# daniel05155/Reinforcement-Learning-in-Music-Generation

Measured on AMD Instinct MI355X. Metric: CW-tokens/sec pretrain fwd+bwd @T=1024, higher is better.
Workload: dtype bf16; 1 GPU; agent_pretrain step (fwd+bwd+clip+Adam), repo dims 512/12/8/2048, synthetic CW tokens (B=512/GPU, T=1024, 7 fields -> 6); per_gpu_batch=512, global_batch=512, seq_len=1024, parallelism=dp1, params=38982227, gemm_table=True

## Files before the change

reinforcement-learning-in-music-generation_amd/csrc/gemm_ln.hip:

```cpp
#include "cwlt_common.h"
#include "cwlt_lds_dma.h"
#include <stdlib.h>

namespace cwlt {
namespace gl {

constexpr int TMR = 128, TNC = 512, BK = 32;
constexpr int NSTAGE = 3;
constexpr int STG = (TMR + TNC) * BK * 2;
constexpr int LDE = TNC + 8;
constexpr int LDS_BYTES = TMR * LDE * 2 > NSTAGE * STG ? TMR * LDE * 2 : NSTAGE * STG;

typedef __bf16 bf16x4 __attribute__((ext_vector_type(4)));

__global__ __launch_bounds__(1024) void gemm_ln_kernel(
    const bf16_t* __restrict__ A, const bf16_t* __restrict__ W, const float* __restrict__ bias,
    const bf16_t* __restrict__ X, const float* __restrict__ gamma, const float* __restrict__ beta,
    bf16_t* __restrict__ S, bf16_t* __restrict__ Y, float* __restrict__ mean, float* __restrict__ rstd, long M, int K,
    long lda, long ldw, float eps, uint32_t thresh, float keep_scale, uint64_t seed,
    const uint64_t* __restrict__ seed_base) {
    extern __shared__ __attribute__((aligned(16))) char lds[];

    const int tid = threadIdx.x, lane = tid & 63;
    const int w = __builtin_amdgcn_readfirstlane(tid >> 6);
    const int wm = w >> 3, wn = w & 7;
    const int l31 = lane & 31, hf = lane >> 5;
    const long m0 = (long)blockIdx.x * TMR;
    const long mrows = min((long)TMR, M - m0);

    const uint64_t abase = (uint64_t)(A + m0 * lda), wbase = (uint64_t)W;
    u32x4_t ars, wrs;
    ars[0] = __builtin_amdgcn_readfirstlane((uint32_t)abase);
    ars[1] = __builtin_amdgcn_readfirstlane((uint32_t)(abase >> 32));
    ars[2] = __builtin_amdgcn_readfirstlane((uint32_t)(((mrows - 1) * lda + K) * 2));
    ars[3] = 0x00020000u;
    wrs[0] = __builtin_amdgcn_readfirstlane((uint32_t)wbase);
    wrs[1] = __builtin_amdgcn_readfirstlane((uint32_t)(wbase >> 32));
    wrs[2] = __builtin_amdgcn_readfirstlane((uint32_t)(((long)(TNC - 1) * ldw + K) * 2));
    wrs[3] = 0x00020000u;
    const int dchunk = (lane & 3) ^ ((lane >> 4) & 3);
    const uint32_t a_voff = ((uint32_t)(16 * (w & 7) + (lane >> 2)) * (uint32_t)lda + dchunk * 8) * 2;
    const uint32_t w_voff = ((uint32_t)(32 * w + (lane >> 2)) * (uint32_t)ldw + dchunk * 8) * 2;
    const uint32_t w_16 = (uint32_t)(16 * ldw * 2);
    const uint32_t lds_a = (uint32_t)(uintptr_t)(lds_void*)lds + (w & 7) * 1024;
    const uint32_t lds_w = (uint32_t)(uintptr_t)(lds_void*)lds + TMR * 64 + w * 2048;
#define GL_DMA_W(stage, step)                                                                                     \
    {                                                                                                             \
        unsigned keep;                                                                                            \
        const uint32_t lw = lds_w + (uint32_t)(stage) * STG;                                                      \
        const uint32_t sk_ = (uint32_t)(step) * (BK * 2), sk2 = sk_ + w_16;                                       \
        asm volatile("s_mov_b32 %0, m0\n\ts_mov_b32 m0, %2\n\ts_nop 4\n\t"                                     \
                     "buffer_load_dwordx4 %1, %3, %4 offen lds\n\t"                                               \
                     "s_add_u32 m0, %2, 0x400\n\ts_nop 0\n\t"                                                    \
                     "buffer_load_dwordx4 %1, %3, %5 offen lds\n\t"                                               \
                     "s_mov_b32 m0, %0"                                                                           \
                     : "=&s"(keep)                                                                                \
                     : "v"(w_voff), "s"(lw), "s"(wrs), "s"(sk_), "s"(sk2)                                         \
                     : "memory", "scc");                                                                          \
    }
#define GL_DMA_A(stage, step) lds_dma_piece(a_voff, ars, lds_a + (uint32_t)(stage) * STG, (uint32_t)(step) * (BK * 2))
#define GL_DMA(stage, step)        \
    {                              \
        if (w < 8) GL_DMA_A(stage, step); \
        GL_DMA_W(stage, step);     \
    }
    const int swz = (l31 >> 2) & 3;
    const int of0 = l31 * 64 + ((hf ^ swz) << 4), of1 = l31 * 64 + (((2 + hf) ^ swz) << 4);
    const int oa = (64 * wm) * 64, ow = TMR * 64 + (64 * wn) * 64;
#define GL_FRAG(p) __builtin_bit_cast(bf16x8, *reinterpret_cast<const uint4*>(p))
#define GL_READ(F, stage, ofh)                                            \
    {                                                                     \
        const char* sb = lds + (stage) * STG;                             \
        F[0] = GL_FRAG(sb + ow + (ofh));                                  \
        F[1] = GL_FRAG(sb + ow + 2048 + (ofh));                           \
        F[2] = GL_FRAG(sb + oa + (ofh));                                  \
        F[3] = GL_FRAG(sb + oa + 2048 + (ofh));                           \
    }
#define GL_MFMA(F)                                                                          \
    {                                                                                       \
        acc[0][0] = __builtin_amdgcn_mfma_f32_32x32x16_bf16(F[0], F[2], acc[0][0], 0, 0, 0); \
        acc[0][1] = __builtin_amdgcn_mfma_f32_32x32x16_bf16(F[1], F[2], acc[0][1], 0, 0, 0); \
        acc[1][0] = __builtin_amdgcn_mfma_f32_32x32x16_bf16(F[0], F[3], acc[1][0], 0, 0, 0); \
        acc[1][1] = __builtin_amdgcn_mfma_f32_32x32x16_bf16(F[1], F[3], acc[1][1], 0, 0, 0); \
    }

    f32x16 acc[2][2];
#pragma unroll
    for (int i = 0; i < 2; ++i)
#pragma unroll
        for (int j = 0; j < 2; ++j)
#pragma unroll
            for (int r = 0; r < 16; ++r) acc[i][j][r] = 0.f;

    const int nstep = K / BK;
    bf16x8 F0[4], F1[4];
    GL_DMA(0, 0);
    GL_DMA(1, 1);
    if (nstep > 2) GL_DMA(2, 2);
    if (nstep > 2) {
        if (w < 8)
            asm volatile("s_waitcnt vmcnt(6)" ::: "memory");
        else
            asm volatile("s_waitcnt vmcnt(4)" ::: "memory");
    } else {
        if (w < 8)
            asm volatile("s_waitcnt vmcnt(3)" ::: "memory");
        else
            asm volatile("s_waitcnt vmcnt(2)" ::: "memory");
    }
    __builtin_amdgcn_s_barrier();
    GL_READ(F0, 0, of0);
    int st = 0;
    for (int s = 0; s < nstep; ++s) {
        const int st1 = st == NSTAGE - 1 ? 0 : st + 1;
        GL_READ(F1, st, of1);
        __builtin_amdgcn_sched_barrier(0);
        GL_MFMA(F0);
        __builtin_amdgcn_sched_barrier(0);
        if (s + 1 < nstep) {
            if (s + 2 < nstep) {
                if (w < 8)
                    asm volatile("s_waitcnt vmcnt(3) lgkmcnt(0)" ::: "memory");
                else
                    asm volatile("s_waitcnt vmcnt(2) lgkmcnt(0)" ::: "memory");
            } else {
                asm volatile("s_waitcnt vmcnt(0) lgkmcnt(0)" ::: "memory");
            }
            __builtin_amdgcn_s_barrier();
            __builtin_amdgcn_sched_barrier(0);
            if (s + 3 < nstep) GL_DMA(st, s + 3);
            GL_READ(F0, st1, of0);
            __builtin_amdgcn_sched_barrier(0);
        }
        GL_MFMA(F1);
        __builtin_amdgcn_sched_barrier(0);
        st = st1;
    }
#undef GL_DMA
#undef GL_DMA_A
#undef GL_DMA_W
#undef GL_FRAG
#undef GL_READ
#undef GL_MFMA

    __syncthreads();
    bf16_t* et = reinterpret_cast<bf16_t*>(lds);
#pragma unroll
    for (int i = 0; i < 2; ++i)
#pragma unroll
        for (int j = 0; j < 2; ++j) {
            const int row = 64 * wm + 32 * i + l31, c0 = 64 * wn + 32 * j;
#pragma unroll
            for (int g = 0; g < 4; ++g) {
                bf16x4 p;
#pragma unroll
                for (int u = 0; u < 4; ++u) p[u] = (__bf16)acc[i][j][4 * g + u];
                *reinterpret_cast<uint2*>(et + row * LDE + c0 + 8 * g + 4 * hf) = __builtin_bit_cast(uint2, p);
            }
        }
    const int ecol = lane * 8;
    uint4 xr[8];
    {
        const __amdgpu_buffer_rsrc_t xrs =
            make_rsrc(X + m0 * TNC, (uint32_t)(mrows * TNC * 2));
#pragma unroll
        for (int i = 0; i < 8; ++i) xr[i] = buf_load16(xrs, ((uint32_t)(w + 16 * i) * TNC + ecol) * 2);
    }
    float gm[8], bt[8], bs[8];
    loadf<8>(gamma + ecol, gm);
    loadf<8>(beta + ecol, bt);
    loadf<8>(bias + ecol, bs);
    __syncthreads();
    if (seed_base) seed += *seed_base;
    const float invN = 1.0f / (float)TNC;
#pragma unroll
    for (int i = 0; i < 8; ++i) {
        const int row = w + 16 * i;
        if (row >= mrows) break;
        const uint4 hv = *reinterpret_cast<const uint4*>(et + row * LDE + ecol);
        float v[8], r[8];
        load8(reinterpret_cast<const bf16_t*>(&hv), v);
        load8(reinterpret_cast<const bf16_t*>(&xr[i]), r);
        const long off = (m0 + row) * TNC + ecol;
        const uint32_t km = thresh ? dropout_mask<8>(seed, (uint64_t)off, thresh) : 0xffffffffu;
        float sum = 0.f;
#pragma unroll
        for (int j = 0; j < 8; ++j) {
            const float a = v[j] + bs[j];
            v[j] = (((km >> j) & 1u) ? a * keep_scale : 0.f) + r[j];
            sum += v[j];
        }
        store8(S + off, v);
        const float mu = wave_sum(sum) * invN;
        float sq = 0.f;
#pragma unroll
        for (int j = 0; j < 8; ++j) {
            const float d = v[j] - mu;
            sq = fmaf(d, d, sq);
        }
        const float rs = rsqrtf(wave_sum(sq) * invN + eps);
        float o[8];
#pragma unroll
        for (int j = 0; j < 8; ++j) o[j] = (v[j] - mu) * rs * gm[j] + bt[j];
        store8(Y + off, o);
        if (lane == 0) {
            mean[m0 + row] = mu;
            rstd[m0 + row] = rs;
        }
    }
}

}
}

extern "C" {

int cwlt_gemm_nt_bias_dropout_add_layernorm(const void* a, const void* w, const float* bias, const void* x,
                                            const float* gamma, const float* beta, void* s, void* y, float* mean,
                                            float* rstd, int64_t M, int N, int K, int64_t lda, int64_t ldw, float eps,
                                            float p, uint64_t seed, const uint64_t* seed_base, void* stream) {
    using namespace cwlt;
    if (M < 0 || N != gl::TNC || K <= 0 || (K % 64) || p < 0.f || p >= 1.f) return CWLT_ERR_ARG;
    if (M == 0) return CWLT_OK;
    if (!a || !w || !bias || !x || !gamma || !beta || !s || !y || !mean || !rstd) return CWLT_ERR_ARG;
    if (((lda | ldw) & 7) || lda < K || ldw < K) return CWLT_ERR_ARG;
    if (((uintptr_t)a | (uintptr_t)w | (uintptr_t)x | (uintptr_t)s | (uintptr_t)y | (uintptr_t)bias | (uintptr_t)gamma |
         (uintptr_t)beta) & 15)
        return CWLT_ERR_ARG;
    if ((int64_t)gl::TMR * lda * 2 >= (1ll << 31) || (int64_t)gl::TNC * ldw * 2 >= (1ll << 31)) return CWLT_ERR_ARG;
    static unsigned long long lds_set = 0;
    int dev = 0;
    if (hipGetDevice(&dev) != hipSuccess) dev = 0;
    if (dev >= 64 || !((lds_set >> dev) & 1ull)) {
        const int e = (int)hipFuncSetAttribute((const void*)gl::gemm_ln_kernel, hipFuncAttributeMaxDynamicSharedMemorySize,
                                               gl::LDS_BYTES);
        if (e) return e;
        if (dev < 64) lds_set |= 1ull << dev;
    }
    const long mtiles = (M + gl::TMR - 1) / gl::TMR;
    hipLaunchKernelGGL(gl::gemm_ln_kernel, dim3((unsigned)mtiles), dim3(1024), gl::LDS_BYTES, (hipStream_t)stream,
                       (const bf16_t*)a, (const bf16_t*)w, bias, (const bf16_t*)x, gamma, beta, (bf16_t*)s, (bf16_t*)y, mean,
                       rstd, (long)M, K, (long)lda, (long)ldw, eps, drop_thresh(p), drop_scale(p), seed, seed_base);
    return (int)hipGetLastError();
}

}
```

Baseline: 3.253 million CW-tokens/s.

## Make fused GEMM+LayerNorm kernel persistent with cross-tile prefetch and dedicated epilogue LDS

Converts the GEMM+bias+dropout+residual+LayerNorm kernel into a persistent kernel launched with at most one block per CU, looping over M tiles with a global DMA step counter. The next tile's A/W loads are issued during the current tile's tail and epilogue, hiding pipeline fill. The epilogue gets its own LDS region and runs in four 32-row quarters, with gamma/beta/bias staged once in LDS and residual loads double-buffered. LDS use per block grows and the wait-count logic across tile boundaries gets more intricate, which risks correctness and occupancy.

```diff
diff --git a/reinforcement-learning-in-music-generation_amd/csrc/gemm_ln.hip b/reinforcement-learning-in-music-generation_amd/csrc/gemm_ln.hip
--- a/reinforcement-learning-in-music-generation_amd/csrc/gemm_ln.hip
+++ b/reinforcement-learning-in-music-generation_amd/csrc/gemm_ln.hip
@@ -9,9 +9,84 @@
 constexpr int NSTAGE = 3;
 constexpr int STG = (TMR + TNC) * BK * 2;
 constexpr int LDE = TNC + 8;
-constexpr int LDS_BYTES = TMR * LDE * 2 > NSTAGE * STG ? TMR * LDE * 2 : NSTAGE * STG;
+constexpr int EQR = 32;
+constexpr int EOFF = NSTAGE * STG;
+constexpr int POFF = EOFF + EQR * LDE * 2;
+constexpr int LDS_BYTES = POFF + 3 * TNC * 4;
 
 typedef __bf16 bf16x4 __attribute__((ext_vector_type(4)));
+
+template <bool FULL>
+__device__ __forceinline__ void glp_quarters(const uint2 (&pk)[2][2][4], char* lds, const bf16_t* __restrict__ X,
+                                             bf16_t* __restrict__ S, bf16_t* __restrict__ Y, long m0, long mrows, int w,
+                                             int lane, float eps, uint32_t thresh, float keep_scale, uint64_t seed,
+                                             float& mus, float& rss) {
+    const int wm = w >> 3, wn = w & 7, l31 = lane & 31, hf = lane >> 5, ecol = lane * 8;
+    const float invN = 1.0f / (float)TNC;
+    bf16_t* et = reinterpret_cast<bf16_t*>(lds + EOFF);
+    const float* pl = reinterpret_cast<const float*>(lds + POFF);
+    const __amdgpu_buffer_rsrc_t xrs = make_rsrc(X + m0 * TNC, (uint32_t)(mrows * TNC * 2));
+    uint4 xr[2][2];
+#pragma unroll
+    for (int k = 0; k < 2; ++k) xr[0][k] = buf_load16(xrs, ((uint32_t)(w + 16 * k) * TNC + ecol) * 2);
+#pragma unroll
+    for (int q = 0; q < 4; ++q) {
+        if (q < 3) {
+#pragma unroll
+            for (int k = 0; k < 2; ++k)
+                xr[(q + 1) & 1][k] = buf_load16(xrs, ((uint32_t)(32 * (q + 1) + w + 16 * k) * TNC + ecol) * 2);
+        }
+        if (q > 0) {
+            asm volatile("s_waitcnt lgkmcnt(0)" ::: "memory");
+            __builtin_amdgcn_s_barrier();
+        }
+        if (wm == (q >> 1)) {
+#pragma unroll
+            for (int j = 0; j < 2; ++j)
+#pragma unroll
+                for (int gq = 0; gq < 4; ++gq)
+                    *reinterpret_cast<uint2*>(et + l31 * LDE + 64 * wn + 32 * j + 8 * gq + 4 * hf) = pk[q & 1][j][gq];
+        }
+        asm volatile("s_waitcnt lgkmcnt(0)" ::: "memory");
+        __builtin_amdgcn_s_barrier();
+#pragma unroll
+        for (int k = 0; k < 2; ++k) {
+            const int row = 32 * q + 16 * k + w;
+            const bool live = FULL || row < mrows;
+            const uint4 hv = *reinterpret_cast<const uint4*>(et + (16 * k + w) * LDE + ecol);
+            float v[8], r[8], gm[8], bt[8], bs[8];
+            loadf<8>(pl + TNC * 2 + ecol, bs);
+            load8(reinterpret_cast<const bf16_t*>(&hv), v);
+            load8(reinterpret_cast<const bf16_t*>(&xr[q & 1][k]), r);
+            const long off = (m0 + row) * TNC + ecol;
+            const uint32_t km = thresh ? dropout_mask<8>(seed, (uint64_t)off, thresh) : 0xffffffffu;
+            float sum = 0.f;
+#pragma unroll
+            for (int j = 0; j < 8; ++j) {
+                const float a = v[j] + bs[j];
+                v[j] = (((km >> j) & 1u) ? a * keep_scale : 0.f) + r[j];
+                sum += v[j];
+            }
+            if (live) store8(S + off, v);
+            const float mu = wave_sum(sum) * invN;
+            float sq = 0.f;
+#pragma unroll
+            for (int j = 0; j < 8; ++j) {
+                const float d = v[j] - mu;
+                sq = fmaf(d, d, sq);
+            }
+            const float rs = rsqrtf(wave_sum(sq) * invN + eps);
+            loadf<8>(pl + ecol, gm);
+            loadf<8>(pl + TNC + ecol, bt);
+            float o[8];
+#pragma unroll
+            for (int j = 0; j < 8; ++j) o[j] = (v[j] - mu) * rs * gm[j] + bt[j];
+            if (live) store8(Y + off, o);
+            mus = lane == 2 * q + k ? mu : mus;
+            rss = lane == 2 * q + k ? rs : rss;
+        }
+    }
+}
 
 __global__ __launch_bounds__(1024) void gemm_ln_kernel(
     const bf16_t* __restrict__ A, const bf16_t* __restrict__ W, const float* __restrict__ bias,
@@ -25,19 +100,32 @@
     const int w = __builtin_amdgcn_readfirstlane(tid >> 6);
     const int wm = w >> 3, wn = w & 7;
     const int l31 = lane & 31, hf = lane >> 5;
-    const long m0 = (long)blockIdx.x * TMR;
-    const long mrows = min((long)TMR, M - m0);
-
-    const uint64_t abase = (uint64_t)(A + m0 * lda), wbase = (uint64_t)W;
+    const long mtiles = (M + TMR - 1) / TMR;
+    const long tstride = (long)gridDim.x * TMR;
+    const int ntl = (int)((mtiles - 1 - blockIdx.x) / gridDim.x) + 1;
+    const int nstep = K / BK;
+    const int G = ntl * nstep;
+    if (seed_base) seed += *seed_base;
+    if (tid < 3 * TNC / 4) {
+        const float* src = tid < TNC / 4 ? gamma : tid < TNC / 2 ? beta : bias;
+        *reinterpret_cast<float4*>(lds + POFF + tid * 16) = load4(src + (tid & (TNC / 4 - 1)) * 4);
+    }
+
+    const uint64_t wbase = (uint64_t)W;
     u32x4_t ars, wrs;
-    ars[0] = __builtin_amdgcn_readfirstlane((uint32_t)abase);
-    ars[1] = __builtin_amdgcn_readfirstlane((uint32_t)(abase >> 32));
-    ars[2] = __builtin_amdgcn_readfirstlane((uint32_t)(((mrows - 1) * lda + K) * 2));
-    ars[3] = 0x00020000u;
     wrs[0] = __builtin_amdgcn_readfirstlane((uint32_t)wbase);
     wrs[1] = __builtin_amdgcn_readfirstlane((uint32_t)(wbase >> 32));
     wrs[2] = __builtin_amdgcn_readfirstlane((uint32_t)(((long)(TNC - 1) * ldw + K) * 2));
     wrs[3] = 0x00020000u;
+#define GLP_ARS(m0_)                                                                                   \
+    {                                                                                                  \
+        const uint64_t ab_ = (uint64_t)(A + (m0_) * lda);                                              \
+        const long mr_ = min((long)TMR, M - (m0_));                                                    \
+        ars[0] = __builtin_amdgcn_readfirstlane((uint32_t)ab_);                                        \
+        ars[1] = __builtin_amdgcn_readfirstlane((uint32_t)(ab_ >> 32));                                \
+        ars[2] = __builtin_amdgcn_readfirstlane((uint32_t)(((mr_ - 1) * lda + K) * 2));                \
+        ars[3] = 0x00020000u;                                                                          \
+    }
     const int dchunk = (lane & 3) ^ ((lane >> 4) & 3);
     const uint32_t a_voff = ((uint32_t)(16 * (w & 7) + (lane >> 2)) * (uint32_t)lda + dchunk * 8) * 2;
     const uint32_t w_voff = ((uint32_t)(32 * w + (lane >> 2)) * (uint32_t)ldw + dchunk * 8) * 2;
@@ -84,131 +172,109 @@
         acc[1][1] = __builtin_amdgcn_mfma_f32_32x32x16_bf16(F[1], F[3], acc[1][1], 0, 0, 0); \
     }
 
-    f32x16 acc[2][2];
-#pragma unroll
-    for (int i = 0; i < 2; ++i)
-#pragma unroll
-        for (int j = 0; j < 2; ++j)
-#pragma unroll
-            for (int r = 0; r < 16; ++r) acc[i][j][r] = 0.f;
-
-    const int nstep = K / BK;
-    bf16x8 F0[4], F1[4];
-    GL_DMA(0, 0);
-    GL_DMA(1, 1);
-    if (nstep > 2) GL_DMA(2, 2);
-    if (nstep > 2) {
+    long pm0 = (long)blockIdx.x * TMR;
+    int pg = 0, pstep = 0, pst = 0;
+    GLP_ARS(pm0);
+#define GLP_ISSUE()                                                 \
+    if (pg < G) {                                                   \
+        GL_DMA(pst, pstep);                                         \
+        ++pg;                                                       \
+        pst = pst == NSTAGE - 1 ? 0 : pst + 1;                      \
+        if (++pstep == nstep) {                                     \
+            pstep = 0;                                              \
+            pm0 += tstride;                                         \
+            if (pg < G) GLP_ARS(pm0);                               \
+        }                                                           \
+    }
+    GLP_ISSUE();
+    GLP_ISSUE();
+    GLP_ISSUE();
+    if (G > 2) {
         if (w < 8)
-            asm volatile("s_waitcnt vmcnt(6)" ::: "memory");
+            asm volatile("s_waitcnt vmcnt(6) lgkmcnt(0)" ::: "memory");
         else
-            asm volatile("s_waitcnt vmcnt(4)" ::: "memory");
+            asm volatile("s_waitcnt vmcnt(4) lgkmcnt(0)" ::: "memory");
     } else {
         if (w < 8)
-            asm volatile("s_waitcnt vmcnt(3)" ::: "memory");
+            asm volatile("s_waitcnt vmcnt(3) lgkmcnt(0)" ::: "memory");
         else
-            asm volatile("s_waitcnt vmcnt(2)" ::: "memory");
+            asm volatile("s_waitcnt vmcnt(2) lgkmcnt(0)" ::: "memory");
     }
     __builtin_amdgcn_s_barrier();
-    GL_READ(F0, 0, of0);
-    int st = 0;
-    for (int s = 0; s < nstep; ++s) {
-        const int st1 = st == NSTAGE - 1 ? 0 : st + 1;
-        GL_READ(F1, st, of1);
-        __builtin_amdgcn_sched_barrier(0);
-        GL_MFMA(F0);
-        __builtin_amdgcn_sched_barrier(0);
-        if (s + 1 < nstep) {
-            if (s + 2 < nstep) {
-                if (w < 8)
-                    asm volatile("s_waitcnt vmcnt(3) lgkmcnt(0)" ::: "memory");
-                else
-                    asm volatile("s_waitcnt vmcnt(2) lgkmcnt(0)" ::: "memory");
-            } else {
-                asm volatile("s_waitcnt vmcnt(0) lgkmcnt(0)" ::: "memory");
+
+    bf16x8 F0[4], F1[4];
+    int st = 0, g = 0;
+    long m0 = (long)blockIdx.x * TMR;
+    for (int t = 0; t < ntl; ++t, m0 += tstride) {
+        f32x16 acc[2][2];
+#pragma unroll
+        for (int i = 0; i < 2; ++i)
+#pragma unroll
+            for (int j = 0; j < 2; ++j)
+#pragma unroll
+                for (int r = 0; r < 16; ++r) acc[i][j][r] = 0.f;
+        GL_READ(F0, st, of0);
+        for (int s = 0; s < nstep; ++s, ++g) {
+            const int st1 = st == NSTAGE - 1 ? 0 : st + 1;
+            GL_READ(F1, st, of1);
+            __builtin_amdgcn_sched_barrier(0);
+            GL_MFMA(F0);
+            __builtin_amdgcn_sched_barrier(0);
+            if (g + 1 < G) {
+                if (t > 0 && s < 2) {
+                    asm volatile("s_waitcnt lgkmcnt(0)" ::: "memory");
+                } else if (g + 2 < G) {
+                    if (w < 8)
+                        asm volatile("s_waitcnt vmcnt(3) lgkmcnt(0)" ::: "memory");
+                    else
+                        asm volatile("s_waitcnt vmcnt(2) lgkmcnt(0)" ::: "memory");
+                } else {
+                    asm volatile("s_waitcnt vmcnt(0) lgkmcnt(0)" ::: "memory");
+                }
+                __builtin_amdgcn_s_barrier();
+                __builtin_amdgcn_sched_barrier(0);
+                GLP_ISSUE();
+                if (s + 1 < nstep) GL_READ(F0, st1, of0);
+                __builtin_amdgcn_sched_barrier(0);
             }
-            __builtin_amdgcn_s_barrier();
+            GL_MFMA(F1);
             __builtin_amdgcn_sched_barrier(0);
-            if (s + 3 < nstep) GL_DMA(st, s + 3);
-            GL_READ(F0, st1, of0);
-            __builtin_amdgcn_sched_barrier(0);
-        }
-        GL_MFMA(F1);
-        __builtin_amdgcn_sched_barrier(0);
-        st = st1;
-    }
+            st = st1;
+        }
+
+        uint2 pk[2][2][4];
+#pragma unroll
+        for (int i = 0; i < 2; ++i)
+#pragma unroll
+            for (int j = 0; j < 2; ++j)
+#pragma unroll
+                for (int gq = 0; gq < 4; ++gq) {
+                    bf16x4 p;
+#pragma unroll
+                    for (int u = 0; u < 4; ++u) p[u] = (__bf16)acc[i][j][4 * gq + u];
+                    pk[i][j][gq] = __builtin_bit_cast(uint2, p);
+                }
+        const long mrows = min((long)TMR, M - m0);
+        float mus = 0.f, rss = 0.f;
+        if (mrows == TMR)
+            glp_quarters<true>(pk, lds, X, S, Y, m0, mrows, w, lane, eps, thresh, keep_scale, seed, mus, rss);
+        else
+            glp_quarters<false>(pk, lds, X, S, Y, m0, mrows, w, lane, eps, thresh, keep_scale, seed, mus, rss);
+        if (lane < 8 && w + 16 * lane < mrows) {
+            mean[m0 + w + 16 * lane] = mus;
+            rstd[m0 + w + 16 * lane] = rss;
+        }
+    }
+#undef GLP_ISSUE
+#undef GLP_ARS
+}
+
 #undef GL_DMA
 #undef GL_DMA_A
 #undef GL_DMA_W
 #undef GL_FRAG
 #undef GL_READ
 #undef GL_MFMA
-
-    __syncthreads();
-    bf16_t* et = reinterpret_cast<bf16_t*>(lds);
-#pragma unroll
-    for (int i = 0; i < 2; ++i)
-#pragma unroll
-        for (int j = 0; j < 2; ++j) {
-            const int row = 64 * wm + 32 * i + l31, c0 = 64 * wn + 32 * j;
-#pragma unroll
-            for (int g = 0; g < 4; ++g) {
-                bf16x4 p;
-#pragma unroll
-                for (int u = 0; u < 4; ++u) p[u] = (__bf16)acc[i][j][4 * g + u];
-                *reinterpret_cast<uint2*>(et + row * LDE + c0 + 8 * g + 4 * hf) = __builtin_bit_cast(uint2, p);
-            }
-        }
-    const int ecol = lane * 8;
-    uint4 xr[8];
-    {
-        const __amdgpu_buffer_rsrc_t xrs =
-            make_rsrc(X + m0 * TNC, (uint32_t)(mrows * TNC * 2));
-#pragma unroll
-        for (int i = 0; i < 8; ++i) xr[i] = buf_load16(xrs, ((uint32_t)(w + 16 * i) * TNC + ecol) * 2);
-    }
-    float gm[8], bt[8], bs[8];
-    loadf<8>(gamma + ecol, gm);
-    loadf<8>(beta + ecol, bt);
-    loadf<8>(bias + ecol, bs);
-    __syncthreads();
-    if (seed_base) seed += *seed_base;
-    const float invN = 1.0f / (float)TNC;
-#pragma unroll
-    for (int i = 0; i < 8; ++i) {
-        const int row = w + 16 * i;
-        if (row >= mrows) break;
-        const uint4 hv = *reinterpret_cast<const uint4*>(et + row * LDE + ecol);
-        float v[8], r[8];
-        load8(reinterpret_cast<const bf16_t*>(&hv), v);
-        load8(reinterpret_cast<const bf16_t*>(&xr[i]), r);
-        const long off = (m0 + row) * TNC + ecol;
-        const uint32_t km = thresh ? dropout_mask<8>(seed, (uint64_t)off, thresh) : 0xffffffffu;
-        float sum = 0.f;
-#pragma unroll
-        for (int j = 0; j < 8; ++j) {
-            const float a = v[j] + bs[j];
-            v[j] = (((km >> j) & 1u) ? a * keep_scale : 0.f) + r[j];
-            sum += v[j];
-        }
-        store8(S + off, v);
-        const float mu = wave_sum(sum) * invN;
-        float sq = 0.f;
-#pragma unroll
-        for (int j = 0; j < 8; ++j) {
-            const float d = v[j] - mu;
-            sq = fmaf(d, d, sq);
-        }
-        const float rs = rsqrtf(wave_sum(sq) * invN + eps);
-        float o[8];
-#pragma unroll
-        for (int j = 0; j < 8; ++j) o[j] = (v[j] - mu) * rs * gm[j] + bt[j];
-        store8(Y + off, o);
-        if (lane == 0) {
-            mean[m0 + row] = mu;
-            rstd[m0 + row] = rs;
-        }
-    }
-}
 
 }
 }
@@ -229,16 +295,24 @@
         return CWLT_ERR_ARG;
     if ((int64_t)gl::TMR * lda * 2 >= (1ll << 31) || (int64_t)gl::TNC * ldw * 2 >= (1ll << 31)) return CWLT_ERR_ARG;
     static unsigned long long lds_set = 0;
+    static int ncu[64];
     int dev = 0;
-    if (hipGetDevice(&dev) != hipSuccess) dev = 0;
+    if (hipGetDevice(&dev) != hipSuccess || dev < 0) dev = 0;
     if (dev >= 64 || !((lds_set >> dev) & 1ull)) {
         const int e = (int)hipFuncSetAttribute((const void*)gl::gemm_ln_kernel, hipFuncAttributeMaxDynamicSharedMemorySize,
                                                gl::LDS_BYTES);
         if (e) return e;
         if (dev < 64) lds_set |= 1ull << dev;
     }
+    int n = dev < 64 ? ncu[dev] : 0;
+    if (!n) {
+        if (hipDeviceGetAttribute(&n, hipDeviceAttributeMultiprocessorCount, dev) != hipSuccess || n < 1) n = 256;
+        if (dev < 64) ncu[dev] = n;
+    }
     const long mtiles = (M + gl::TMR - 1) / gl::TMR;
-    hipLaunchKernelGGL(gl::gemm_ln_kernel, dim3((unsigned)mtiles), dim3(1024), gl::LDS_BYTES, (hipStream_t)stream,
+    const long grid = mtiles < n ? mtiles : n;
+    if ((mtiles / grid + 1) * (K / gl::BK) >= (1ll << 31)) return CWLT_ERR_ARG;
+    hipLaunchKernelGGL(gl::gemm_ln_kernel, dim3((unsigned)grid), dim3(1024), gl::LDS_BYTES, (hipStream_t)stream,
                        (const bf16_t*)a, (const bf16_t*)w, bias, (const bf16_t*)x, gamma, beta, (bf16_t*)s, (bf16_t*)y, mean,
                        rstd, (long)M, K, (long)lda, (long)ldw, eps, drop_thresh(p), drop_scale(p), seed, seed_base);
     return (int)hipGetLastError();
```

New measurement: 3.265 million CW-tokens/s, median of 6. About the same (+0.4%).
